# zjucsxxd/hdr2yuv

Hardware: AMD Instinct MI355X
Metric: Mpixels/s, 4K RGB->YUV420 PQ convert path (in-memory, HBM-resident) (higher is better)
Workload: dtype f32+f64

## Files before the change

hdr2yuv_amd/csrc/h2y_device.h:

```cpp
#ifndef H2Y_DEVICE_H
#define H2Y_DEVICE_H

#include <hip/hip_runtime.h>
#include <stdint.h>

#include "h2y_kernels.h"
#include "h2y_math.h"

using namespace h2y;

#define WAVE 64

__device__ __forceinline__ float wave_min(float v)
{
#pragma unroll
    for (int o = 32; o > 0; o >>= 1) v = fminf(v, __shfl_xor(v, o, WAVE));
    return v;
}
__device__ __forceinline__ float wave_max(float v)
{
#pragma unroll
    for (int o = 32; o > 0; o >>= 1) v = fmaxf(v, __shfl_xor(v, o, WAVE));
    return v;
}
// ... 219 lines not shown
{
    const uint32_t xb = f2bits(x);
    const bool cand = slow && (xb - 0x00800000u) < (lo_bits - 0x00800000u);
    if (__builtin_expect(__builtin_amdgcn_ballot_w64(cand) != 0 && ext != nullptr, 0)) {
        const uint32_t idx = cand ? (xb >> H2Y_PQ_LOW_BITS) - H2Y_PQX_SEG_BASE : 0u;
        const pq_ext_rec *X = reinterpret_cast<const pq_ext_rec *>(ext);
        const pq_recA a = X[idx].a;
        const pq_recB b = X[idx].b;
        const double d = pq_poly(xb, a, b);
        v = cand ? (float)d : v;
        slow = cand ? pq_ambiguous(d) : slow;
    }
    return v;
}

static __device__ __attribute__((noinline)) float tf_to_linear_careful(int cls, float v) { return tf_to_linear(cls, v); }
static __device__ __attribute__((noinline)) float tf_from_linear_careful(int cls, float v) { return tf_from_linear(cls, v); }

#define H2Y_PIPE_RUNTIME 0
#define H2Y_PIPE_PQ_IDENT 1
#define H2Y_PIPE_PQ_NORM 2
#define H2Y_PIPE_NONE 6
#define H2Y_PIPE_TFN 7

template <int PIPE> __device__ __forceinline__ float norm1(const pix_params &pp, int c, float v)
{
    const bool conv = PIPE == H2Y_PIPE_RUNTIME ? pp.convert_transfer != 0 : true;
    const bool ident = PIPE == H2Y_PIPE_RUNTIME ? pp.norm_identity : PIPE == H2Y_PIPE_PQ_IDENT;
    return (conv && !ident) ? (v - pp.offset[c]) / pp.range[c] : v;
}
// ... 172 lines not shown
```

hdr2yuv_amd/csrc/h2y_fir_fused.hip:

```cpp
#include <hip/hip_runtime.h>
#include <stdint.h>

#include <stdio.h>

#include "h2y_device.h"

#define FF_THREADS 1024
#ifndef FF_BUFFER_STORE
#define FF_BUFFER_STORE 1
#endif
#define FF_OWN_LANES H2Y_FF_OWN_LANES
#define FF_HALO ((64 - FF_OWN_LANES) / 2)

template <bool RAW> struct ff_rows;
template <> struct ff_rows<false> { float g0[4], b0[4], r0[4], g1[4], b1[4], r1[4]; };
template <> struct ff_rows<true> { uint32_t g0[2], b0[2], r0[2], g1[2], b1[2], r1[2]; };
template <int IN_KIND> __device__ __forceinline__ void ff_load(const void *p, uint32_t q, float (&d)[4]) { in_traits<IN_KIND>::load4q(p, q, d); }
template <int IN_KIND> __device__ __forceinline__ void ff_load(const void *p, uint32_t q, uint32_t (&d)[2])
{
    const u32x2 t = gload_nt<u32x2>(p, q);
    d[0] = t.x; d[1] = t.y;
}
__device__ __forceinline__ uint32_t ff_pk_min_h(uint32_t a, uint32_t b) { uint32_t r; asm("v_pk_min_f16 %0, %1, %2" : "=v"(r) : "v"(a), "v"(b)); return r; }
__device__ __forceinline__ uint32_t ff_pk_max_h(uint32_t a, uint32_t b) { uint32_t r; asm("v_pk_max_f16 %0, %1, %2" : "=v"(r) : "v"(a), "v"(b)); return r; }
// ... 155 lines not shown
        const uint32_t qx = (uint32_t)min(max(qxu, 0), (int32_t)WQ - 1);
        const bool own = lane >= (uint32_t)FF_HALO && lane < (uint32_t)FF_HALO + FF_OWN_LANES && qxu < (int32_t)WQ;
#if FF_BUFFER_STORE
        const uint32_t qx_store = own ? qx : 0x20000000u;
        const __amdgpu_buffer_rsrc_t out_rsrc = __builtin_amdgcn_make_buffer_rsrc(io.out, 0, (int)((npix + 2u * ncb) * 2u), 0x00020000);
#endif
        ff_edges e;
        e.any = __builtin_amdgcn_readfirstlane((uint32_t)(strip == 0u) | (uint32_t)(strip + 1u == nst));
        e.left0 = qxu == 0;
        e.left1 = qxu == 1;
        e.right0 = qxu == (int32_t)WQ - 1;

        mm6 mm;
        mm.reset();
        uint32_t flagged = 0;
        uint64_t low_m = 0;
        ff_hist hb[2], hr[2];
        hb[0].fill(0u); hb[1].fill(0u); hr[0].fill(0u); hr[1].fill(0u);

        constexpr bool RAW = TIER == FF_TIER_LUT16;
        constexpr int NREG = RAW ? 2 : 4;
        uint32_t hmn[3] = {0x7C007C00u, 0x7C007C00u, 0x7C007C00u}, hmx[3] = {0u, 0u, 0u};
        ff_rows<RAW> v;
        uint32_t q0 = 2u * (s_begin < H2 - 1u ? s_begin : H2 - 1u) * WQ + qx;
        ff_load<IN_KIND>(io.in[0], q0, v.g0); ff_load<IN_KIND>(io.in[1], q0, v.b0); ff_load<IN_KIND>(io.in[2], q0, v.r0);
        ff_load<IN_KIND>(io.in[0], q0 + WQ, v.g1); ff_load<IN_KIND>(io.in[1], q0 + WQ, v.b1); ff_load<IN_KIND>(io.in[2], q0 + WQ, v.r1);
#pragma unroll
        for (int j = 0; j < NREG; j++) asm volatile("" ::"v"(v.g0[j]), "v"(v.b0[j]), "v"(v.r0[j]), "v"(v.g1[j]), "v"(v.b1[j]), "v"(v.r1[j]));

        for (uint32_t s = s_begin; s <= s_end; s++) {
// ... 64 lines not shown
                    Y[col] = f2bits(gv[col]) >> 21; Cb[col] = f2bits(bv[col]) >> 21; Cr[col] = f2bits(rv[col]) >> 21;
                    continue;
#endif
                    const float Gn = norm1<PIPE>(pp, 0, gv[col]), Bn = norm1<PIPE>(pp, 1, bv[col]), Rn = norm1<PIPE>(pp, 2, rv[col]);
                    const pq_rec1 cg = pq_t1_fetch(Gn, s_t1), cb = pq_t1_fetch(Bn, s_t1), cr = pq_t1_fetch(Rn, s_t1);
                    __builtin_amdgcn_sched_barrier(0);
                    float mg, mb, mr;
                    const float g = pix_scale(pq_t1_eval_m(Gn, cg, &mg), pp.mulY, pp.addY);
                    const float b = pix_scale(pq_t1_eval_m(Bn, cb, &mb), pp.mulC, pp.addC);
                    const float rr = pix_scale(pq_t1_eval_m(Rn, cr, &mr), pp.mulC, pp.addC);
                    bool ra, rb;
                    pix_matrix_t1<MODE>(pp, sn, g, b, rr, pq_t1_unsure3(mg, mb, mr), Y[col], Cb[col], Cr[col], &ra, &rb);
                    const uint64_t fm = __builtin_amdgcn_ballot_w64(ra) | __builtin_amdgcn_ballot_w64(rb);
                    if (__builtin_expect(fm != 0, 0)) {
                        const bool ug = pq_t1_unsure(mg), ub = pq_t1_unsure(mb), ur = pq_t1_unsure(mr);
                        uint32_t Y2, Cb2, Cr2;
                        const bool fl = ((fm >> lane) & 1u) != 0;
                        float g2 = g, b2 = b, r2 = rr;
                        bool un = false;
                        if (__builtin_amdgcn_ballot_w64(fl & ug) != 0) {
                            bool sl;
                            const float t = pq_ext_inline(Gn, pq_fast(Gn, sA, sB, &sl), sl, pp.pq_ext);
                            g2 = (fl & ug) ? pix_scale(t, pp.mulY, pp.addY) : g2;
                            un |= fl & ug & sl;
                        }
                        if (__builtin_amdgcn_ballot_w64(fl & ub) != 0) {
                            bool sl;
                            const float t = pq_ext_inline(Bn, pq_fast(Bn, sA, sB, &sl), sl, pp.pq_ext);
                            b2 = (fl & ub) ? pix_scale(t, pp.mulC, pp.addC) : b2;
                            un |= fl & ub & sl;
                        }
                        if (__builtin_amdgcn_ballot_w64(fl & ur) != 0) {
                            bool sl;
                            const float t = pq_ext_inline(Rn, pq_fast(Rn, sA, sB, &sl), sl, pp.pq_ext);
                            r2 = (fl & ur) ? pix_scale(t, pp.mulC, pp.addC) : r2;
                            un |= fl & ur & sl;
                        }
                        bool um;
                        pix_matrix<MODE, false>(pp, g2, b2, r2, Y2, Cb2, Cr2, &um);
                        un |= um;
                        if (__builtin_expect(fl & un, 0)) {
                            const ycc k = pixel_careful<MODE>(&s_pp, Gn, Bn, Rn);
                            Y2 = k.y; Cb2 = k.cb; Cr2 = k.cr;
                        }
                        Y[col] = fl ? Y2 : Y[col];
                        Cb[col] = fl ? Cb2 - pp.half_m1 : Cb[col];
                        Cr[col] = fl ? Cr2 - pp.half_m1 : Cr[col];
                        flagged += (uint32_t)__popcll(fm);
                        if (PIPE == H2Y_PIPE_PQ_IDENT) low_m |= __builtin_amdgcn_ballot_w64(fl && min3f(Gn, Bn, Rn) <= -1.0f);
                    }
                    }
                }
                yp[row][0] = pix_yuv_clamp<true>(pp, Y[0], false) | (pix_yuv_clamp<true>(pp, Y[1], false) << 16);
                yp[row][1] = pix_yuv_clamp<true>(pp, Y[2], false) | (pix_yuv_clamp<true>(pp, Y[3], false) << 16);
#if defined(H2Y_EXP_NOCOMPUTE) && H2Y_EXP_NOCOMPUTE >= 2
                n_cb[row][0] = Cb[0]; n_cb[row][1] = Cb[2]; n_cr[row][0] = Cr[0]; n_cr[row][1] = Cr[2];
#else
                ff_hstage<TIER == FF_TIER_T1>(Cb, e, maxcv, hk0, n_cb[row][0], n_cb[row][1]);
                ff_hstage<TIER == FF_TIER_T1>(Cr, e, maxcv, hk0, n_cr[row][0], n_cr[row][1]);
#endif
                if (row == 0) {
                    ff_load<IN_KIND>(io.in[0], q0n, v.g0);
                    ff_load<IN_KIND>(io.in[1], q0n, v.b0);
                    ff_load<IN_KIND>(io.in[2], q0n, v.r0);
// ... 47 lines not shown
        if constexpr (RAW) {
#pragma unroll
            for (int c = 0; c < 3; c++) {
                mm.lo[c] = fminf(ff_half_to_float(hmn[c] & 0xFFFFu), ff_half_to_float(hmn[c] >> 16));
                mm.hi[c] = fmaxf(ff_half_to_float(hmx[c] & 0xFFFFu), ff_half_to_float(hmx[c] >> 16));
                mm.lo[c] = mm.lo[c] > 65504.0f ? 3.402823466e+38f : mm.lo[c];
                mm.hi[c] = mm.hi[c] <= 0.0f ? 1.175494351e-38f : mm.hi[c];
            }
        }
        asm volatile("" : "+s"(ap));
        const uint32_t f_end = __builtin_amdgcn_readfirstlane(u / ap->units_per_frame);
        const size_t slot = (size_t)u;
        wave_store_mm(mm, ap->partial + slot * 6);
        if (lane == 0) {
            ap->redo_count[slot] = flagged >> 3;
            if (PIPE == H2Y_PIPE_PQ_IDENT && ap->low_flag && low_m != 0) ap->low_flag[f_end] = 1u;
        }
    }
    if (a.block_clock && (threadIdx.x & (WAVE - 1)) == 0) atomicMax(&a.block_clock[2 * blockIdx.x + 1], (unsigned long long)wall_clock64());
#ifdef H2Y_BLOCK_TIMES
    if ((threadIdx.x & (WAVE - 1)) == 0) atomicMax(&g_ff_block_times[2 * blockIdx.x + 1], (unsigned long long)wall_clock64());
#endif
}

typedef void (*firf_fn)(firf_args);
template <int IN_KIND> static firf_fn pick_firf(int mode, int pipe)
{
    if (mode == H2Y_MODE_YCBCR)
        return pipe == H2Y_PIPE_PQ_IDENT ? k_fir_fused<IN_KIND, H2Y_MODE_YCBCR, H2Y_PIPE_PQ_IDENT, FF_TIER_T1>
                                         : k_fir_fused<IN_KIND, H2Y_MODE_YCBCR, H2Y_PIPE_PQ_NORM, FF_TIER_T1>;
// ... 16 lines not shown
```

hdr2yuv_amd/csrc/h2y_forward.hip:

```cpp
#include "h2y_shim.h"
#include "h2y_plan.h"

namespace {

const double kT1DenseShare = 0.007;
const double kFirSyncMaxFlagged = 0.004;
const int kT1SkipBatches = 32;
const int kT1SkipBatchesMax = 1024;

int tmp_depth_of(const h2y_desc *d) { return d->in_sample_type == H2Y_SAMPLE_U16 ? d->src_bit_depth : d->dst_bit_depth; }

}

void derive_params(const h2y_desc *d, pix_params *pp, bool stage_matrix_only)
{
    memset(pp, 0, sizeof *pp);
    const int tmp_depth = tmp_depth_of(d);
    const clip_limits tc = make_clip(tmp_depth, d->dst_full_range);
    const clip_limits oc = make_clip(d->dst_bit_depth, d->dst_full_range);
    pp->src_tf = tf_class(d->src_transfer);
    pp->dst_tf = tf_class(d->dst_transfer);
    if (d->src_transfer == d->dst_transfer) pp->convert_transfer = 0;
    else pp->convert_transfer = (pp->src_tf == H2Y_TF_LINEAR && pp->dst_tf == H2Y_TF_PQ) ? 1 : 2;
    pp->src_fn = pp->dst_fn = -1;
// ... 43 lines not shown
        }
    }
    pix_limits_finish(pp);
}

namespace {

void t1_begin_batch(h2y_ctx *ctx)
{
    ctx->cur_skip_t1 = ctx->t1_skip > 0;
    if (ctx->cur_skip_t1) ctx->t1_skip--;
}
void t1_end_batch(h2y_ctx *ctx, const h2y_desc *d, const frame_stats *fs, int n)
{
    if (!ctx->b->was_t1 || n < 1) return;
    uint64_t redone = 0;
    for (int f = 0; f < n; f++) redone += fs[f].redone;
    const uint64_t tiles = (uint64_t)n * make_geom(d->width, d->height, 1024).tiles;
    if (!strcmp(ctx->last_name, "k_fir_fused")) ctx->fir_flag_share = tiles ? (double)redone / (double)tiles : 0.0;
    {
        const size_t at = ctx->last_variant.find(" flagged=");
        if (at != std::string::npos) ctx->last_variant.erase(at);
        char note[48];
        snprintf(note, sizeof note, " flagged=%.5f", tiles ? (double)redone / (double)tiles : 0.0);
        ctx->last_variant += note;
    }
    if (ctx->opt_t1_steer && (double)redone > kT1DenseShare * (double)tiles) {
        ctx->t1_skip_len = ctx->t1_skip_len ? (ctx->t1_skip_len < kT1SkipBatchesMax ? 2 * ctx->t1_skip_len : kT1SkipBatchesMax) : kT1SkipBatches;
        ctx->t1_skip = ctx->t1_skip_len;
    } else ctx->t1_skip_len = 0;
}

fused_variant pick_variant(const h2y_ctx *ctx, const h2y_desc *d, const pix_params &pp, int out_kind, const assumed_stats *known, t1_sens *sn)
{
    memset(sn, 0, sizeof *sn);
    fused_variant v;
    v.in_kind = in_kind_of(d);
    v.out_kind = out_kind;
    v.mode = pp.mode;
    v.narrow = (d->width % 4) != 0;
    v.even_h = (d->height & 1) == 0;
    v.pipe = 0;
// ... 154 lines not shown
    fa.src_bit_depth = d->src_bit_depth;
    fa.redo_count = nullptr;
    fa.low_flag = nullptr;
    fa.check = 0;
    fa.assumed = nullptr;
    fa.publish = nullptr;
    fa.block_clock = nullptr;
    fa.grid = 0;
    fa.xcd_time = nullptr;
    return fa;
}
final_args launch_final(const h2y_ctx *ctx, const frames_run &r, int f0, int nblk, bool redo, bool low, bool clocks, int grid)
{
    final_args fa = stats_final(ctx, r.d, nblk, ctx->b->fs_out + r.fstats_offset + f0);
    fa.redo_count = redo ? ctx->b->d_redo : nullptr;
    fa.low_flag = low ? ctx->b->d_low : nullptr;
    fa.check = r.check ? 1 : 0;
    fa.assumed = r.d_assumed;
    fa.block_clock = clocks ? ctx->b->d_clock : nullptr;
    fa.grid = grid;
    static_assert(sizeof(frame_stats) >= 8 * sizeof(float), "the XCD run times ride in one frame_stats entry");
    fa.xcd_time = reinterpret_cast<float *>(ctx->b->fs_out + r.fstats_offset + r.n);
    return fa;
}

int stage_unit_rows(h2y_ctx *ctx, const std::vector<uint32_t> &rows)
{
    batch_state *b = ctx->b;
    const size_t units = rows.size();
    if (b->unit_rows_cap < units) {
// ... 16 lines not shown

int launch_fir_fused(h2y_ctx *ctx, const frames_run &r, const fir_plan &p)
{
    batch_state *b = ctx->b;
    const h2y_desc *d = r.d;
    const int n = r.n, grid = p.grid;
    const fused_variant &var = r.var;
    const bool ident = var.pipe == 4 || var.pipe == 3;
    const uint32_t upf = p.strips * p.segments;
    b->was_t1 = true;
    for (int i = 0; i < n; i++) b->h_frames[(size_t)ctx->slot_base + i] = r.frames[i];
    int rc = stage_frames(ctx, 0, n);
    if (rc) return rc;
    rc = ensure(ctx, b->d_partial, b->partial_cap, (size_t)n * upf * 6 * sizeof(float));
    if (rc) return rc;
    rc = ensure(ctx, b->d_redo, b->redo_cap, (size_t)n * upf * sizeof(uint32_t));
    if (rc) return rc;
    if (ident && (rc = ensure_low(ctx, n))) return rc;
    if (r.check) b->approx_min = ident;
    firf_args fa;
    fa.frames = b->d_frames + ctx->slot_base;
    fa.n_frames = n;
    fa.width = (uint32_t)d->width;
    fa.height = (uint32_t)d->height;
    fa.wq = p.wq;
    fa.n_strips = p.strips;
    fa.n_seg = p.segments;
    fa.seg_rows = p.seg_rows;
    fa.units_per_frame = upf;
    fa.total_units = (uint32_t)p.units;
    const int fsync = ctx->opt_fir_sync >= 0 ? ctx->opt_fir_sync : (ctx->fir_flag_share > kFirSyncMaxFlagged ? 0 : 1);
    fa.sync_mask = fsync > 0 ? (uint32_t)fsync - 1u : ~0u;
    fa.table = ctx->d_table;
    fa.table1 = ctx->d_table1;
    fa.lut16 = ctx->d_lut16;
    fa.sn = r.sn;
    fa.partial = b->d_partial;
    fa.redo_count = b->d_redo;
    fa.low_flag = ident ? b->d_low : nullptr;
    fa.assumed = r.d_assumed;
    fa.pp = r.pp;
    fa.unit_rows = nullptr;
    fa.block_clock = nullptr;
    fa.mix_xcds = p.mix_xcds;
    const bool clocks = p.full && r.time_it;
    const balance bal = balance_of(ctx);
    const bool weigh = fir_weigh(p, bal, ctx->ffb_have);
    double work[8] = {0, 0, 0, 0, 0, 0, 0, 0};
    if (weigh || clocks) {
        double sp[8];
        for (int x = 0; x < 8; x++) sp[x] = bal.speed(x, ctx->ffb_speed);
        std::vector<uint32_t> rows;
        fir_unit_rows(p, n, weigh, sp, rows, work);
// ... 67 lines not shown
    a.pp.tf_ext[0] = sf ? ctx->d_tfn_ext[sf] : nullptr;
    a.pp.tf_ext[1] = df ? ctx->d_tfn_ext[df] : nullptr;
    return 0;
}

int launch_fused(h2y_ctx *ctx, const frames_run &r, const geom &g, const launch_plan &l, int f0, bool first_launch, bool yuvp2)
{
    batch_state *b = ctx->b;
    const h2y_desc *d = r.d;
    const fused_variant &var = r.var;
    const int nf = l.frames, grid = l.grid, groups = l.groups;
    const int waves = h2y_fused_threads(var) / 64;
    int rc = ensure(ctx, b->d_partial, b->partial_cap, (size_t)nf * grid * waves * 6 * sizeof(float));
    if (rc) return rc;
    const bool t1 = var.pipe == 4 || var.pipe == 5;
    if (t1 && (rc = ensure(ctx, b->d_redo, b->redo_cap, (size_t)nf * grid * waves * sizeof(uint32_t)))) return rc;
    const bool approx = var.pipe == 4;
    if (approx && (rc = ensure_low(ctx, nf))) return rc;
    if (r.check) b->approx_min = approx;
    const uint32_t *d_slice_ranges = nullptr;
    slice_plan sl;
    for (int x = 0; x < 8; x++) sl.work[x] = 1;
    if (l.xcd_layout && ctx->opt_bal_mode != 1) {
        const balance bal = balance_of(ctx);
        double sp[8];
        for (int x = 0; x < 8; x++) sp[x] = bal.speed(x, ctx->bal_have ? ctx->bal_speed : nullptr);
        const block_speeds bs{ctx->opt_bal_mode == 0 && ctx->opt_bal_blocks, ctx->bal_bgrid, ctx->bal_bgroups, &ctx->bal_bspeed};
        make_slice_plan(sl, l, g.tiles, sp, bs, t1, ctx->opt_tail);
        if ((rc = publish_ranges(ctx, sl.r, first_launch, &d_slice_ranges))) return rc;
    }
    const bool clocks = l.xcd_layout && r.time_it;
// ... 2 lines not shown
    a.xcd_layout = l.xcd_layout ? 1u : 0u;
    a.block_clock = clocks ? b->d_clock : nullptr;
    a.slice_ranges = d_slice_ranges;
    a.range_stride = sl.range_stride;
    a.tail_ctr = nullptr;
    a.tail_slices = 0;
    if (sl.tail_on && d_slice_ranges) {
        if (!b->d_tail) {
            HIP_TRY(ctx, hipMalloc((void **)&b->d_tail, 16 * H2Y_TAIL_WORDS * sizeof(uint32_t)));
            HIP_TRY(ctx, hipMemsetAsync(b->d_tail, 0, 16 * H2Y_TAIL_WORDS * sizeof(uint32_t), ctx->stream));
        }
        a.tail_ctr = b->d_tail;
        a.tail_slices = sl.slices;
    }
    a.redo_count = t1 ? b->d_redo : nullptr;
    a.low_flag = approx ? b->d_low : nullptr;
    a.frames = b->d_frames + ctx->slot_base + f0;
    a.n_frames = nf;
    a.width = d->width;
    a.height = d->height;
    a.wq = g.wq;
    a.wq_magic = g.wq_magic;
    a.tiles_per_frame = g.tiles;
    a.chunks_per_frame = g.chunks;
    a.groups = (uint32_t)groups;
    a.table = ctx->d_table;
    a.table_src = a.table_dst = nullptr;
    a.lut16 = ctx->d_lut16;
    a.table1 = ctx->d_table1;
    a.sn = r.sn;
// ... 562 lines not shown
```

hdr2yuv_amd/csrc/h2y_kernels.h:

```cpp
#ifndef H2Y_KERNELS_H
#define H2Y_KERNELS_H

#include <hip/hip_runtime.h>
#include <stdint.h>

#include "h2y_math.h"
#include "h2y_walk.h"

#ifndef H2Y_FUSED_THREADS
#define H2Y_FUSED_THREADS 512
#endif
#ifndef H2Y_FUSED_MINWAVES
#define H2Y_FUSED_MINWAVES 4
#endif

#ifndef H2Y_LOOP_THREADS
#define H2Y_LOOP_THREADS 1024
#endif

#define H2Y_LUT16_N 16384

enum { H2Y_IN_F32 = 0, H2Y_IN_F16 = 1, H2Y_IN_U16 = 2 };
enum { H2Y_OUT_420BOX = 0, H2Y_OUT_444 = 1, H2Y_OUT_444TMP = 2 };

// ... 1 lines not shown
    const void *in[3];
    uint16_t *out;
    union {
        uint16_t *tmp_cb;
        uint16_t *yuv;
    };
    uint16_t *tmp_cr;
};

struct frame_stats {
    float mm[6];
    int32_t floor_[3];
    int32_t ceil_[3];
    int32_t mismatch;
    uint32_t redone;
};

struct assumed_stats {
    int32_t floor_[3];
    int32_t ceil_[3];
};

struct fused_args {
    const frame_io *frames;
    int n_frames;
    uint32_t width, height;
    uint32_t wq;
    uint32_t wq_magic;
    uint32_t tiles_per_frame;
    uint32_t chunks_per_frame;
    uint32_t groups;
    uint32_t xcd_layout;
    unsigned long long *block_clock;
    const uint32_t *slice_ranges;
    uint32_t *tail_ctr = nullptr;
    uint32_t tail_slices = 0;
    uint32_t range_stride = 0;
    const void *table;
    const void *table_src, *table_dst;
    const float *lut16;
    const void *table1;
    h2y::t1_sens sn;
    uint32_t tiles_magic;
    float *partial;
    uint32_t *redo_count;
    uint32_t *low_flag;
    const assumed_stats *assumed;
    h2y::pix_params pp;
};

struct fused_variant {
    int in_kind, out_kind, mode;
    int pipe;
    bool narrow;
    bool even_h;
    bool t1_ok = false;
    bool cols8 = false;
};

struct stats_args {
    const void *in[3];
    size_t npix;
    int vec_ok;
    float *partial;
};

struct final_args {
    const float *partial;
    const uint32_t *redo_count;
    uint32_t *low_flag;
    int nblk;
    frame_stats *out;
    int is_u16, src_bit_depth;
    int check;
    const assumed_stats *assumed;
    assumed_stats *publish;
    unsigned long long *block_clock;
    int grid;
    float *xcd_time;
    float *block_time = nullptr;
    uint32_t *tail_ctr = nullptr;
    int tail_n = 0;
};

// ... 32 lines not shown
    uint32_t width, height;
    uint32_t wq;
    uint32_t n_strips;
    uint32_t n_seg, seg_rows;
    const uint32_t *unit_rows;
    unsigned long long *block_clock;
    uint32_t mix_xcds;
    uint32_t units_per_frame;
    uint32_t total_units;
    uint32_t sync_mask;
    const void *table, *table1;
    const float *lut16;
    h2y::t1_sens sn;
    float *partial;
    uint32_t *redo_count;
    uint32_t *low_flag;
    const assumed_stats *assumed;
    h2y::pix_params pp;
};

enum { UP_REPLICATE = 0, UP_FIR = 1, UP_FIR_TL = 2 };
struct up_args {
    const uint16_t *src0, *src1;
    uint16_t *dst0, *dst1;
    int width, height;
    int algorithm;
    float fmin, fmax;
};

struct inv420_args {
// ... 356 lines not shown
```

hdr2yuv_amd/csrc/h2y_kernels.hip:

```cpp
#include <hip/hip_runtime.h>
#include <stdint.h>
#include <string.h>
#include <stdio.h>

#include "h2y_math.h"
#include "h2y_kernels.h"
#include "h2y_walk.h"
#include "h2y_device.h"

struct tile_pos {
    uint32_t tt;
    uint32_t q0, q1;
    bool row1;
};
__device__ __forceinline__ tile_pos tile_locate(uint32_t tt, uint32_t W, uint32_t H, uint32_t WQ, uint32_t magic)
{
    tile_pos t;
    uint32_t cg;
    (void)udiv_magic(tt, WQ, magic, cg);
    t.tt = tt;
    t.q0 = 2u * tt - cg;
    t.row1 = tt < WQ * (H >> 1);
    t.q1 = t.row1 ? t.q0 + WQ : t.q0;
    return t;
// ... 672 lines not shown
    for (; fw.f < fw.n_frames; fw.advance(), fo++) {
        const int f = fw.f;
        const bool dyn = tail_ctr != nullptr && !fw.has_next();
        const bool dyn_n = tail_ctr != nullptr && fw.has_next() && f + 2 * (int)fw.NG >= fw.n_frames;
        uint32_t dyn_t0 = 0;
        asm volatile("" : "+s"(ap));
        const frame_io *const frames = ap->frames;
        const frame_io io = uniform_io(frames + f);
        typedef const __attribute__((address_space(4))) frame_io *frame_cptr;
        const frame_cptr io_next_p = (frame_cptr)(uintptr_t)(frames + (fw.has_next() ? f + (int)fw.NG : f));
        mm6 mm;
        mm.reset();
        const uint32_t id_base = (uint32_t)f * a.tiles_per_frame;
        uint32_t flagged_f = 0;
        uint32_t flagged_px = 0;
        wave_deal deal, deal_n;
        if (ranged) {
            deal.set_range(r_first, r_count);
            deal_n.set_range(r_first, r_count);
        } else {
            deal.set(fw, fw.k0, H2Y_T1_THREADS / WAVE);
            deal_n.set(fw, fw.k0_n, H2Y_T1_THREADS / WAVE);
        }
        if (dyn) {
            if (!hold) {
                tick = wave_claim(&s_tq[H2Y_TAIL_QLEN + 2], s_scratch, true);
                hold = dyn_tile0(tick, dyn_t0);
            } else dyn_t0 = dyn_carry;
        } else if (!hold) {
            tick = wave_claim(&s_claim[fo], s_scratch, true);
// ... 119 lines not shown
                        if (row == 1) { Y[col] = o.yp0[col >> 1] >> (16 * (col & 1)) & 0xFFFFu; Cb[col] = sb[col >> 1] >> 1; Cr[col] = sr[col >> 1] >> 1; continue; }
#endif
                        const float Gn = norm1<PIPE>(pp, 0, gv[col]);
                        const float Bn = norm1<PIPE>(pp, 1, bv[col]);
                        const float Rn = norm1<PIPE>(pp, 2, rv[col]);
                        const pq_rec1 cg = pq_t1_fetch(Gn, s_t1), cb = pq_t1_fetch(Bn, s_t1), cr = pq_t1_fetch(Rn, s_t1);
                        __builtin_amdgcn_sched_barrier(0);
                        float mg, mb, mr;
                        const float g = pix_scale(pq_t1_eval_m(Gn, cg, &mg), pp.mulY, pp.addY);
                        const float b = pix_scale(pq_t1_eval_m(Bn, cb, &mb), pp.mulC, pp.addC);
                        const float r = pix_scale(pq_t1_eval_m(Rn, cr, &mr), pp.mulC, pp.addC);
                        bool ra, rb;
                        pix_matrix_t1<MODE>(pp, sn, g, b, r, pq_t1_unsure3(mg, mb, mr), Y[col], Cb[col], Cr[col], &ra, &rb);
                        const uint64_t fm = __builtin_amdgcn_ballot_w64(ra) | __builtin_amdgcn_ballot_w64(rb);
                        if (__builtin_expect(fm != 0, 0)) {
                            const bool fl = ((fm >> lane) & 1u) != 0;
                            const bool ug = pq_t1_unsure(mg), ub = pq_t1_unsure(mb), ur = pq_t1_unsure(mr);
                            float g2 = g, b2 = b, r2 = r;
                            bool un = false;
                            if (__builtin_amdgcn_ballot_w64(fl & ug) != 0) {
                                bool sl;
                                const float t = pq_ext_inline(Gn, pq_fast(Gn, s_t2, sB2, &sl), sl, pp.pq_ext);
                                g2 = (fl & ug) ? pix_scale(t, pp.mulY, pp.addY) : g2;
                                un |= fl & ug & sl;
                            }
                            if (__builtin_amdgcn_ballot_w64(fl & ub) != 0) {
                                bool sl;
                                const float t = pq_ext_inline(Bn, pq_fast(Bn, s_t2, sB2, &sl), sl, pp.pq_ext);
                                b2 = (fl & ub) ? pix_scale(t, pp.mulC, pp.addC) : b2;
                                un |= fl & ub & sl;
                            }
                            if (__builtin_amdgcn_ballot_w64(fl & ur) != 0) {
                                bool sl;
                                const float t = pq_ext_inline(Rn, pq_fast(Rn, s_t2, sB2, &sl), sl, pp.pq_ext);
                                r2 = (fl & ur) ? pix_scale(t, pp.mulC, pp.addC) : r2;
                                un |= fl & ur & sl;
                            }
                            uint32_t Y2, Cb2, Cr2;
                            bool um;
                            pix_matrix<MODE, false>(pp, g2, b2, r2, Y2, Cb2, Cr2, &um);
                            Y[col] = fl ? Y2 : Y[col];
                            Cb[col] = fl ? Cb2 - pp.half_m1 : Cb[col];
                            Cr[col] = fl ? Cr2 - pp.half_m1 : Cr[col];
                            redo_m |= __builtin_amdgcn_ballot_w64(fl & (un | um));
                            flagged_px += (uint32_t)__popcll(fm);
                        }
                        asm volatile("" : "+s"(redo_m));
                    }
                    row_pack<OUT_KIND, true, true>(pp, row, Y, Cb, Cr, o, sb, sr);
                }
                tile_store<OUT_KIND>(io, t, W, H, o);
                v = nx;
                t_cur = t2;
                {
                    const uint64_t m = redo_m;
                    const bool flagged = ((m >> lane) & 1u) != 0;
                    const uint32_t below = __builtin_amdgcn_mbcnt_hi((uint32_t)(m >> 32), __builtin_amdgcn_mbcnt_lo((uint32_t)m, 0u));
                    my_list[flagged ? n_redo + below : (uint32_t)(H2Y_REDO_CAP - 1)] = id_base + umin32(tt, a.tiles_per_frame - 1u);
                    n_redo = __builtin_amdgcn_readfirstlane(n_redo + (uint32_t)__popcll(m));
                    flagged_f = __builtin_amdgcn_readfirstlane(flagged_f + (uint32_t)__popcll(m));
// ... 1 lines not shown
                more = kind == 1;
                tick = tick2;
                if (dyn) dyn_t0 = dyn_t0_next;
            } while (more && n_redo < WAVE);
            if (n_redo >= WAVE) {
                n_redo -= WAVE;
#ifndef H2Y_SKIP_REDO
                redo_pass<IN_KIND, OUT_KIND, MODE, PIPE>(&s_rc, &s_pp, s_t2, my_list, n_redo, WAVE);
                have = false;
#endif
            }
        }
        asm volatile("" : "+s"(ap));
        wave_store_mm(mm, ap->partial + walk_slot(fw, H2Y_T1_THREADS / WAVE) * 6);
        if (ap->redo_count && lane == 0) ap->redo_count[walk_slot(fw, H2Y_T1_THREADS / WAVE)] = flagged_f + (flagged_px >> 3);
    }
#ifdef H2Y_BLOCK_TIMES
    if (blockIdx.x < 4 && lane == 0) g_block_times[2 * (800 + blockIdx.x * 16 + wave)] = wall_clock64();
#endif
    if (n_redo) redo_pass<IN_KIND, OUT_KIND, MODE, PIPE>(&s_rc, &s_pp, s_t2, my_list, 0u, n_redo);
    block_clock_end(a);
#ifdef H2Y_BLOCK_TIMES
    __syncthreads();
    if (threadIdx.x == 0) g_block_times[2 * blockIdx.x + 1] = wall_clock64();
#endif
    (void)lane;
}

typedef _Float16 h2 __attribute__((ext_vector_type(2)));
__device__ __forceinline__ uint32_t pk_min_h(uint32_t a, uint32_t b)
// ... 251 lines not shown
            IN::load4(a.in[c], i * 4, v);
            mm.add2(c, v[0], v[1]);
            mm.add2(c, v[2], v[3]);
        }
    }
    for (size_t i = n4 * 4 + (size_t)blockIdx.x * blockDim.x + threadIdx.x; i < n; i += stride)
#pragma unroll
        for (int c = 0; c < 3; c++) mm.add(c, IN::load1(a.in[c], i));
    block_store_mm<H2Y_FUSED_THREADS / WAVE>(mm, s_red, a.partial + (size_t)blockIdx.x * 6);
}

#define H2Y_FINAL_THREADS 1024
__global__ __launch_bounds__(H2Y_FINAL_THREADS) void k_stats_final(final_args a)
{
    __shared__ float s_red[(H2Y_FINAL_THREADS / WAVE) * 6];
    __shared__ uint32_t s_cnt;
    __shared__ int s_start[1024], s_finish[1024], s_min[8];
    const int f = blockIdx.x;
    const float *p = a.partial + (size_t)f * a.nblk * 6;
    frame_stats *out = a.out + f;
    mm6 mm;
    mm.reset();
    uint32_t cnt = 0;
    for (int i = threadIdx.x; i < a.nblk; i += blockDim.x) {
#pragma unroll
        for (int c = 0; c < 3; c++) {
            mm.lo[c] = fminf(mm.lo[c], p[i * 6 + 2 * c]);
            mm.hi[c] = fmaxf(mm.hi[c], p[i * 6 + 2 * c + 1]);
        }
        if (a.redo_count) cnt += a.redo_count[(size_t)f * a.nblk + i];
    }
    int as_floor[3] = {0, 0, 0}, as_ceil[3] = {0, 0, 0};
    uint32_t low = 0;
    if (threadIdx.x == 0) {
        if (a.check)
            for (int c = 0; c < 3; c++) { as_floor[c] = a.assumed->floor_[c]; as_ceil[c] = a.assumed->ceil_[c]; }
        if (a.low_flag) low = a.low_flag[f];
    }
    const bool clocks = a.block_clock && f == 0;
    const int nb = min(a.grid, 1024);
    if (clocks) {
        const unsigned long long ref = a.block_clock[0];
        for (int b = (int)threadIdx.x; b < a.grid; b += (int)blockDim.x) {
            if (b < nb) {
                s_start[b] = (int)(long long)(a.block_clock[2 * b] - ref);
                s_finish[b] = (int)(long long)(a.block_clock[2 * b + 1] - ref);
            }
            a.block_clock[2 * b + 1] = 0ull;
        }
    }
    if (a.tail_ctr && f == 0)
        for (int i = (int)threadIdx.x; i < a.tail_n; i += (int)blockDim.x) a.tail_ctr[i] = 0u;
    if (threadIdx.x == 0) s_cnt = 0;
    __syncthreads();
    if (a.redo_count) {
#pragma unroll
        for (int o = WAVE / 2; o > 0; o >>= 1) cnt += (uint32_t)__shfl_xor((int)cnt, o, WAVE);
        if ((threadIdx.x & (WAVE - 1)) == 0) atomicAdd(&s_cnt, cnt);
    }
    block_store_mm<H2Y_FINAL_THREADS / WAVE>(mm, s_red, out->mm);
    if (threadIdx.x == 0) {
        out->redone = a.redo_count ? s_cnt : 0u;
        int bad = 0;
        for (int c = 0; c < 3; c++) {
            float lo = s_red[2 * c], hi = s_red[2 * c + 1];
            int fl, ce;
            if (a.is_u16) {
                fl = (int)lo;
                ce = (int)hi;
                const int D = 1 << (a.src_bit_depth - 8), SMin = D * 16;
                const int YMax = 219 * D + SMin, CMax = 224 * D + SMin;
                if (ce < YMax && ce > (YMax * 3) / 4) ce = YMax;
                if (ce < CMax && ce > (CMax * 3) / 4) ce = CMax;
            } else {
                lo = fminf(fmaxf(lo, -2147483648.0f), 2147483520.0f);
                hi = fminf(fmaxf(hi, -2147483648.0f), 2147483520.0f);
                fl = (int)lo;
// ... 379 lines not shown
```

hdr2yuv_amd/csrc/h2y_math.h:

```cpp
#ifndef H2Y_MATH_H
#define H2Y_MATH_H

#if defined(H2Y_EXP_NOCOMPUTE) || defined(H2Y_HALF_COMPUTE) || defined(H2Y_SKIP_REDO) || defined(H2Y_EXP_NOSTATS) || defined(H2Y_EXP_NOCONFLICT) || \
    defined(H2Y_BLOCK_TIMES)
#ifndef H2Y_EXPERIMENT
#error "timing-experiment variant requested without -DH2Y_EXPERIMENT: this would build a product library with wrong bytes or debug output"
#endif
#endif

#include <stdint.h>
#include <vector>

#if defined(__HIPCC__)
#define H2Y_FN __host__ __device__ __forceinline__
#define H2Y_FN_NOINLINE __host__ __device__ inline __attribute__((noinline))
#else
#define H2Y_FN inline
#define H2Y_FN_NOINLINE inline __attribute__((noinline))
#endif

namespace h2y {

H2Y_FN uint32_t f2bits(float f) { return __builtin_bit_cast(uint32_t, f); }
H2Y_FN float bits2f(uint32_t u) { return __builtin_bit_cast(float, u); }
// ... 778 lines not shown
                dd num = dd_add(ev[j], dd{-ev[j - 1].hi, -ev[j - 1].lo});
                ev[j] = dd_div(num, dd{wn[j] - wn[j - lvl], 0.0});
            }
        const dd q2 = ev[2];
        const dd q1 = dd_add(ev[1], dd_mul_d(q2, -(wn[0] + wn[1])));
        const dd q0 = dd_add(dd_add(ev[0], dd_mul_d(ev[1], -wn[0])), dd_mul_d(q2, wn[0] * wn[1]));
        const double r = (double)(2 << H2Y_T1_SEG_BITS);
        const float c = (float)q0.hi;
        o.cb = bits2f(f2bits(c) + 1u);
        o.c0 = (float)((((q0.hi - (double)c) + q0.lo) * inv_u - 0.5) + (double)H2Y_T1_DELTA);
        o.c1 = (float)(q1.hi * r * inv_u);
        o.c2 = (float)(q2.hi * r * r * inv_u);
    }
    T[0] = T[H2Y_T1_NSEG + 1] = nan_rec;
}
enum : int { H2Y_MODE_IDENTITY = 0, H2Y_MODE_YDZDX = 1, H2Y_MODE_YCBCR = 2, H2Y_MODE_YPQRS = 3, H2Y_MODE_YUVP2 = 4 };

struct pix_params {
    int convert_transfer;
    int src_tf, dst_tf;
    int src_fn, dst_fn;
    int norm_identity;
    float offset[3], range[3];
    float mulY, addY, mulC, addC;
    int mode;
    double kr, kg, kb;
    double dcb, dcr;
    double inv_dcb, inv_dcr;
    float P, Q, RR, S;
    uint32_t half_m1;
// ... 163 lines not shown
    Cro = (uint32_t)sat_i32_f64(qr);
    const uint32_t fb = (uint32_t)(d2bits(fract_f64(qb)) >> 32), fr = (uint32_t)(d2bits(fract_f64(qr)) >> 32);
    const bool y_unsafe = !(__builtin_fabsf(fract_f32(ylike) - 0.5f) < sn.ty);
    const bool guard = vunc & (((fb - sn.cb_lo) >= sn.cb_span) | ((fr - sn.cr_lo) >= sn.cr_span));
    *ra = guard | (vunc & y_unsafe);
    *rb = false;
}
template <int MODE>
H2Y_FN bool pix_matrix_t1(const pix_params &pp, const t1_sens &sn, float G, float B, float R, bool vunc, uint32_t &Yo,
                          uint32_t &Cbo, uint32_t &Cro)
{
    bool ra, rb;
    pix_matrix_t1<MODE>(pp, sn, G, B, R, vunc, Yo, Cbo, Cro, &ra, &rb);
    return ra | rb;
}

H2Y_FN uint32_t hiword_of(double v) { return (uint32_t)(d2bits(v) >> 32); }
inline bool t1_chroma_in_range(const pix_params &pp)
{
    const double vhi = pq_exact_dd(dd{(double)H2Y_T1_DOMAIN_HI, 0.0}).hi * (1.0 + 1e-6), vlo = pq_exact_dd(dd{(double)H2Y_T1_DOMAIN_LO, 0.0}).hi * (1.0 - 1e-6);
    auto span = [&](double mul, double add, double *lo, double *hi) {
        const double a = add + mul * vlo, b = add + mul * vhi;
        *lo = (a < b ? a : b) - 1e-3 - 1e-6 * __builtin_fabs(a < b ? a : b);
        *hi = (a < b ? b : a) + 1e-3 + 1e-6 * __builtin_fabs(a < b ? b : a);
    };
    double glo, ghi, clo, chi;
    span(pp.mulY, pp.addY, &glo, &ghi);
    span(pp.mulC, pp.addC, &clo, &chi);
    double qlo[2], qhi[2];
    if (pp.mode == H2Y_MODE_YCBCR) {
// ... 180 lines not shown
```

hdr2yuv_amd/csrc/h2y_shim.h:

```cpp
#pragma once

#include <hip/hip_runtime.h>

#include <cmath>
#include <cstdarg>
#include <cstdio>
#include <cstdlib>
#include <algorithm>
#include <cstring>
#include <memory>
#include <new>
#include <string>
#include <vector>

#include "../../include/hdr2yuv_hip.h"
#include "h2y_kernels.h"
#include "h2y_math.h"

using namespace h2y;

#pragma GCC visibility push(hidden)

struct clip_limits {
    uint32_t minCV, maxCV, minVR, maxVR, minVRC, maxVRC, Half;
// ... 72 lines not shown
    int planes_check(h2y_ctx *ctx, const h2y_desc *d) const;
    uint64_t payload_bytes() const;
    uintptr_t align() const;
    hipError_t launch(const h2y_ctx *ctx, const payload_frame *frames, int n) const;
    const char *kernel() const;
    std::string variant() const;
};

struct batch_state {
    frame_io *d_frames = nullptr, *h_frames = nullptr;
    size_t frames_cap = 0;
    std::vector<frame_io> dev_frames;
    float *d_partial = nullptr;
    size_t partial_cap = 0;
    uint32_t *d_redo = nullptr;
    size_t redo_cap = 0;
    uint32_t *d_low = nullptr;
    size_t low_cap = 0;
    bool approx_min = false;
    unsigned long long *d_clock = nullptr;
    size_t clock_cap = 0;
    int bal_slot = 0;
    bool bal_pending = false;
    double bal_work[8] = {1, 1, 1, 1, 1, 1, 1, 1};
    uint32_t *h_ranges = nullptr, *hd_ranges = nullptr;
    uint32_t *d_tail = nullptr;
    float *h_btime = nullptr, *hd_btime = nullptr;
    int bal_grid = 0, bal_groups = 0;
    std::vector<double> bal_bwork;
    std::vector<uint32_t> range_slot[2];
// ... 323 lines not shown
```

Measured before the change: 375,900.

## Settle dark-pixel flagged lanes with a float PQ approximation before slow path

Adds a float-only PQ evaluation for very dark inputs (log2/exp2 polynomials plus a Newton reciprocal) that settles flagged pixels in the tier-1 and fused FIR kernels. When the result's error bound is safe, these pixels skip the slow double-precision extension path and are no longer counted as redone. The dark counts are tracked separately and reported through stats_final. The host steering heuristic changes to use a separate FIR dense threshold that ignores dark-settled pixels, so fewer batches fall back away from tier-1. It adds register pressure and extra ballots on the rare flagged path.

```diff
diff --git a/hdr2yuv_amd/csrc/h2y_device.h b/hdr2yuv_amd/csrc/h2y_device.h
--- a/hdr2yuv_amd/csrc/h2y_device.h
+++ b/hdr2yuv_amd/csrc/h2y_device.h
@@ -257,6 +257,32 @@
     return v;
 }
 
+template <int MODE>
+__device__ __forceinline__ uint64_t t1_dark_settle(const pix_params &pp, const t1_sens &sn, uint64_t fm, uint32_t lane, float Gn, float Bn, float Rn,
+                                                   bool ug, bool ub, bool ur, float g, float b, float r, uint32_t &Y, uint32_t &Cb, uint32_t &Cr,
+                                                   uint64_t *settled)
+{
+    const bool fl = ((fm >> lane) & 1u) != 0;
+    const bool dg = pq_is_dark(Gn), db = pq_is_dark(Bn), dr = pq_is_dark(Rn);
+    *settled = 0;
+    if (__builtin_amdgcn_ballot_w64(fl & (dg | db | dr)) == 0) return fm;
+    float gA = g, bA = b, rA = r;
+    if (__builtin_amdgcn_ballot_w64(fl & dg) != 0) gA = dg ? pix_scale(pq_dark(Gn), pp.mulY, pp.addY) : g;
+    if (__builtin_amdgcn_ballot_w64(fl & db) != 0) bA = db ? pix_scale(pq_dark(Bn), pp.mulC, pp.addC) : b;
+    if (__builtin_amdgcn_ballot_w64(fl & dr) != 0) rA = dr ? pix_scale(pq_dark(Rn), pp.mulC, pp.addC) : r;
+    uint32_t Y2, Cb2, Cr2;
+    bool ra, rb;
+    pix_matrix_t1<MODE>(pp, sn, gA, bA, rA, true, Y2, Cb2, Cr2, &ra, &rb);
+    const bool other = (ug & !dg) | (ub & !db) | (ur & !dr);
+    const bool fin = fl & (dg | db | dr) & !other & !(ra | rb) & t1_chroma_raw_ok(pp, Cb2) & t1_chroma_raw_ok(pp, Cr2);
+    Y = fin ? Y2 : Y;
+    Cb = fin ? Cb2 : Cb;
+    Cr = fin ? Cr2 : Cr;
+    const uint64_t fin_m = __builtin_amdgcn_ballot_w64(fin);
+    *settled = fin_m;
+    return fm & ~fin_m;
+}
+
 static __device__ __attribute__((noinline)) float tf_to_linear_careful(int cls, float v) { return tf_to_linear(cls, v); }
 static __device__ __attribute__((noinline)) float tf_from_linear_careful(int cls, float v) { return tf_from_linear(cls, v); }
 
diff --git a/hdr2yuv_amd/csrc/h2y_fir_fused.hip b/hdr2yuv_amd/csrc/h2y_fir_fused.hip
--- a/hdr2yuv_amd/csrc/h2y_fir_fused.hip
+++ b/hdr2yuv_amd/csrc/h2y_fir_fused.hip
@@ -193,6 +193,7 @@
         mm6 mm;
         mm.reset();
         uint32_t flagged = 0;
+        uint32_t dark_px = 0;
         uint64_t low_m = 0;
         ff_hist hb[2], hr[2];
         hb[0].fill(0u); hb[1].fill(0u); hr[0].fill(0u); hr[1].fill(0u);
@@ -287,8 +288,12 @@
                     const uint64_t fm = __builtin_amdgcn_ballot_w64(ra) | __builtin_amdgcn_ballot_w64(rb);
                     if (__builtin_expect(fm != 0, 0)) {
                         const bool ug = pq_t1_unsure(mg), ub = pq_t1_unsure(mb), ur = pq_t1_unsure(mr);
+                        uint64_t dark_m;
+                        const uint64_t fm2 = t1_dark_settle<MODE>(pp, sn, fm, lane, Gn, Bn, Rn, ug, ub, ur, g, b, rr, Y[col], Cb[col], Cr[col], &dark_m);
+                        dark_px += (uint32_t)__popcll(dark_m);
+                        if (fm2 != 0) {
                         uint32_t Y2, Cb2, Cr2;
-                        const bool fl = ((fm >> lane) & 1u) != 0;
+                        const bool fl = ((fm2 >> lane) & 1u) != 0;
                         float g2 = g, b2 = b, r2 = rr;
                         bool un = false;
                         if (__builtin_amdgcn_ballot_w64(fl & ug) != 0) {
@@ -319,8 +324,9 @@
                         Y[col] = fl ? Y2 : Y[col];
                         Cb[col] = fl ? Cb2 - pp.half_m1 : Cb[col];
                         Cr[col] = fl ? Cr2 - pp.half_m1 : Cr[col];
-                        flagged += (uint32_t)__popcll(fm);
+                        flagged += (uint32_t)__popcll(fm2);
                         if (PIPE == H2Y_PIPE_PQ_IDENT) low_m |= __builtin_amdgcn_ballot_w64(fl && min3f(Gn, Bn, Rn) <= -1.0f);
+                        }
                     }
                     }
                 }
@@ -398,6 +404,7 @@
         wave_store_mm(mm, ap->partial + slot * 6);
         if (lane == 0) {
             ap->redo_count[slot] = flagged >> 3;
+            if (ap->dark_count) ap->dark_count[slot] = ((flagged + dark_px) >> 3) - (flagged >> 3);
             if (PIPE == H2Y_PIPE_PQ_IDENT && ap->low_flag && low_m != 0) ap->low_flag[f_end] = 1u;
         }
     }
diff --git a/hdr2yuv_amd/csrc/h2y_forward.hip b/hdr2yuv_amd/csrc/h2y_forward.hip
--- a/hdr2yuv_amd/csrc/h2y_forward.hip
+++ b/hdr2yuv_amd/csrc/h2y_forward.hip
@@ -3,7 +3,9 @@
 
 namespace {
 
-const double kT1DenseShare = 0.007;
+const double kT1DenseShare = 0.010;
+const double kFirDenseShare = 0.003;
+const double kFirDarkKeep = 0.10;
 const double kFirSyncMaxFlagged = 0.004;
 const int kT1SkipBatches = 32;
 const int kT1SkipBatchesMax = 1024;
@@ -81,18 +83,22 @@
 void t1_end_batch(h2y_ctx *ctx, const h2y_desc *d, const frame_stats *fs, int n)
 {
     if (!ctx->b->was_t1 || n < 1) return;
-    uint64_t redone = 0;
-    for (int f = 0; f < n; f++) redone += fs[f].redone;
+    uint64_t redone = 0, dark = 0;
+    for (int f = 0; f < n; f++) { redone += fs[f].redone; dark += fs[f].dark; }
     const uint64_t tiles = (uint64_t)n * make_geom(d->width, d->height, 1024).tiles;
-    if (!strcmp(ctx->last_name, "k_fir_fused")) ctx->fir_flag_share = tiles ? (double)redone / (double)tiles : 0.0;
+    if (!strcmp(ctx->last_name, "k_fir_fused")) ctx->fir_flag_share = tiles ? (double)(redone + dark) / (double)tiles : 0.0;
     {
         const size_t at = ctx->last_variant.find(" flagged=");
         if (at != std::string::npos) ctx->last_variant.erase(at);
-        char note[48];
-        snprintf(note, sizeof note, " flagged=%.5f", tiles ? (double)redone / (double)tiles : 0.0);
+        char note[80];
+        int len = snprintf(note, sizeof note, " flagged=%.5f", tiles ? (double)(redone + dark) / (double)tiles : 0.0);
+        if (tiles && 2000 * dark >= tiles) snprintf(note + len, sizeof note - (size_t)len, " dark=%.3f", (double)dark / (double)tiles);
         ctx->last_variant += note;
     }
-    if (ctx->opt_t1_steer && (double)redone > kT1DenseShare * (double)tiles) {
+    const bool fir = !strcmp(ctx->last_name, "k_fir_fused");
+    const bool dense = fir ? (double)redone > kFirDenseShare * (double)tiles && (double)dark < kFirDarkKeep * (double)tiles
+                           : (double)redone > kT1DenseShare * (double)tiles;
+    if (ctx->opt_t1_steer && dense) {
         ctx->t1_skip_len = ctx->t1_skip_len ? (ctx->t1_skip_len < kT1SkipBatchesMax ? 2 * ctx->t1_skip_len : kT1SkipBatchesMax) : kT1SkipBatches;
         ctx->t1_skip = ctx->t1_skip_len;
     } else ctx->t1_skip_len = 0;
@@ -277,6 +283,7 @@
 {
     final_args fa = stats_final(ctx, r.d, nblk, ctx->b->fs_out + r.fstats_offset + f0);
     fa.redo_count = redo ? ctx->b->d_redo : nullptr;
+    fa.dark_count = redo ? ctx->b->d_dark : nullptr;
     fa.low_flag = low ? ctx->b->d_low : nullptr;
     fa.check = r.check ? 1 : 0;
     fa.assumed = r.d_assumed;
@@ -323,8 +330,9 @@
     if (rc) return rc;
     rc = ensure(ctx, b->d_partial, b->partial_cap, (size_t)n * upf * 6 * sizeof(float));
     if (rc) return rc;
-    rc = ensure(ctx, b->d_redo, b->redo_cap, (size_t)n * upf * sizeof(uint32_t));
-    if (rc) return rc;
+    rc = ensure(ctx, b->d_redo, b->redo_cap, 2 * (size_t)n * upf * sizeof(uint32_t));
+    if (rc) return rc;
+    b->d_dark = b->d_redo + (size_t)n * upf;
     if (ident && (rc = ensure_low(ctx, n))) return rc;
     if (r.check) b->approx_min = ident;
     firf_args fa;
@@ -346,6 +354,7 @@
     fa.sn = r.sn;
     fa.partial = b->d_partial;
     fa.redo_count = b->d_redo;
+    fa.dark_count = b->d_dark;
     fa.low_flag = ident ? b->d_low : nullptr;
     fa.assumed = r.d_assumed;
     fa.pp = r.pp;
@@ -443,7 +452,8 @@
     int rc = ensure(ctx, b->d_partial, b->partial_cap, (size_t)nf * grid * waves * 6 * sizeof(float));
     if (rc) return rc;
     const bool t1 = var.pipe == 4 || var.pipe == 5;
-    if (t1 && (rc = ensure(ctx, b->d_redo, b->redo_cap, (size_t)nf * grid * waves * sizeof(uint32_t)))) return rc;
+    if (t1 && (rc = ensure(ctx, b->d_redo, b->redo_cap, 2 * (size_t)nf * grid * waves * sizeof(uint32_t)))) return rc;
+    if (t1) b->d_dark = b->d_redo + (size_t)nf * grid * waves;
     const bool approx = var.pipe == 4;
     if (approx && (rc = ensure_low(ctx, nf))) return rc;
     if (r.check) b->approx_min = approx;
@@ -476,6 +486,7 @@
         a.tail_slices = sl.slices;
     }
     a.redo_count = t1 ? b->d_redo : nullptr;
+    a.dark_count = t1 ? b->d_dark : nullptr;
     a.low_flag = approx ? b->d_low : nullptr;
     a.frames = b->d_frames + ctx->slot_base + f0;
     a.n_frames = nf;
diff --git a/hdr2yuv_amd/csrc/h2y_kernels.h b/hdr2yuv_amd/csrc/h2y_kernels.h
--- a/hdr2yuv_amd/csrc/h2y_kernels.h
+++ b/hdr2yuv_amd/csrc/h2y_kernels.h
@@ -39,6 +39,7 @@
     int32_t ceil_[3];
     int32_t mismatch;
     uint32_t redone;
+    uint32_t dark;
 };
 
 struct assumed_stats {
@@ -69,6 +70,7 @@
     uint32_t tiles_magic;
     float *partial;
     uint32_t *redo_count;
+    uint32_t *dark_count = nullptr;
     uint32_t *low_flag;
     const assumed_stats *assumed;
     h2y::pix_params pp;
@@ -93,6 +95,7 @@
 struct final_args {
     const float *partial;
     const uint32_t *redo_count;
+    const uint32_t *dark_count = nullptr;
     uint32_t *low_flag;
     int nblk;
     frame_stats *out;
@@ -155,6 +158,7 @@
     h2y::t1_sens sn;
     float *partial;
     uint32_t *redo_count;
+    uint32_t *dark_count = nullptr;
     uint32_t *low_flag;
     const assumed_stats *assumed;
     h2y::pix_params pp;
diff --git a/hdr2yuv_amd/csrc/h2y_kernels.hip b/hdr2yuv_amd/csrc/h2y_kernels.hip
--- a/hdr2yuv_amd/csrc/h2y_kernels.hip
+++ b/hdr2yuv_amd/csrc/h2y_kernels.hip
@@ -710,6 +710,7 @@
         const uint32_t id_base = (uint32_t)f * a.tiles_per_frame;
         uint32_t flagged_f = 0;
         uint32_t flagged_px = 0;
+        uint32_t dark_px = 0;
         wave_deal deal, deal_n;
         if (ranged) {
             deal.set_range(r_first, r_count);
@@ -859,8 +860,12 @@
                         pix_matrix_t1<MODE>(pp, sn, g, b, r, pq_t1_unsure3(mg, mb, mr), Y[col], Cb[col], Cr[col], &ra, &rb);
                         const uint64_t fm = __builtin_amdgcn_ballot_w64(ra) | __builtin_amdgcn_ballot_w64(rb);
                         if (__builtin_expect(fm != 0, 0)) {
-                            const bool fl = ((fm >> lane) & 1u) != 0;
                             const bool ug = pq_t1_unsure(mg), ub = pq_t1_unsure(mb), ur = pq_t1_unsure(mr);
+                            uint64_t dark_m;
+                            const uint64_t fm2 = t1_dark_settle<MODE>(pp, sn, fm, lane, Gn, Bn, Rn, ug, ub, ur, g, b, r, Y[col], Cb[col], Cr[col], &dark_m);
+                            dark_px += (uint32_t)__popcll(dark_m);
+                            if (fm2 != 0) {
+                            const bool fl = ((fm2 >> lane) & 1u) != 0;
                             float g2 = g, b2 = b, r2 = r;
                             bool un = false;
                             if (__builtin_amdgcn_ballot_w64(fl & ug) != 0) {
@@ -888,7 +893,8 @@
                             Cb[col] = fl ? Cb2 - pp.half_m1 : Cb[col];
                             Cr[col] = fl ? Cr2 - pp.half_m1 : Cr[col];
                             redo_m |= __builtin_amdgcn_ballot_w64(fl & (un | um));
-                            flagged_px += (uint32_t)__popcll(fm);
+                            flagged_px += (uint32_t)__popcll(fm2);
+                            }
                         }
                         asm volatile("" : "+s"(redo_m));
                     }
@@ -920,6 +926,7 @@
         asm volatile("" : "+s"(ap));
         wave_store_mm(mm, ap->partial + walk_slot(fw, H2Y_T1_THREADS / WAVE) * 6);
         if (ap->redo_count && lane == 0) ap->redo_count[walk_slot(fw, H2Y_T1_THREADS / WAVE)] = flagged_f + (flagged_px >> 3);
+        if (ap->dark_count && lane == 0) ap->dark_count[walk_slot(fw, H2Y_T1_THREADS / WAVE)] = ((flagged_px + dark_px) >> 3) - (flagged_px >> 3);
     }
 #ifdef H2Y_BLOCK_TIMES
     if (blockIdx.x < 4 && lane == 0) g_block_times[2 * (800 + blockIdx.x * 16 + wave)] = wall_clock64();
@@ -1201,14 +1208,14 @@
 __global__ __launch_bounds__(H2Y_FINAL_THREADS) void k_stats_final(final_args a)
 {
     __shared__ float s_red[(H2Y_FINAL_THREADS / WAVE) * 6];
-    __shared__ uint32_t s_cnt;
+    __shared__ uint32_t s_cnt, s_dark;
     __shared__ int s_start[1024], s_finish[1024], s_min[8];
     const int f = blockIdx.x;
     const float *p = a.partial + (size_t)f * a.nblk * 6;
     frame_stats *out = a.out + f;
     mm6 mm;
     mm.reset();
-    uint32_t cnt = 0;
+    uint32_t cnt = 0, dark = 0;
     for (int i = threadIdx.x; i < a.nblk; i += blockDim.x) {
 #pragma unroll
         for (int c = 0; c < 3; c++) {
@@ -1216,6 +1223,7 @@
             mm.hi[c] = fmaxf(mm.hi[c], p[i * 6 + 2 * c + 1]);
         }
         if (a.redo_count) cnt += a.redo_count[(size_t)f * a.nblk + i];
+        if (a.dark_count) dark += a.dark_count[(size_t)f * a.nblk + i];
     }
     int as_floor[3] = {0, 0, 0}, as_ceil[3] = {0, 0, 0};
     uint32_t low = 0;
@@ -1238,16 +1246,22 @@
     }
     if (a.tail_ctr && f == 0)
         for (int i = (int)threadIdx.x; i < a.tail_n; i += (int)blockDim.x) a.tail_ctr[i] = 0u;
-    if (threadIdx.x == 0) s_cnt = 0;
+    if (threadIdx.x == 0) s_cnt = s_dark = 0;
     __syncthreads();
     if (a.redo_count) {
 #pragma unroll
         for (int o = WAVE / 2; o > 0; o >>= 1) cnt += (uint32_t)__shfl_xor((int)cnt, o, WAVE);
         if ((threadIdx.x & (WAVE - 1)) == 0) atomicAdd(&s_cnt, cnt);
+    }
+    if (a.dark_count) {
+#pragma unroll
+        for (int o = WAVE / 2; o > 0; o >>= 1) dark += (uint32_t)__shfl_xor((int)dark, o, WAVE);
+        if ((threadIdx.x & (WAVE - 1)) == 0) atomicAdd(&s_dark, dark);
     }
     block_store_mm<H2Y_FINAL_THREADS / WAVE>(mm, s_red, out->mm);
     if (threadIdx.x == 0) {
         out->redone = a.redo_count ? s_cnt : 0u;
+        out->dark = a.dark_count ? s_dark : 0u;
         int bad = 0;
         for (int c = 0; c < 3; c++) {
             float lo = s_red[2 * c], hi = s_red[2 * c + 1];
diff --git a/hdr2yuv_amd/csrc/h2y_math.h b/hdr2yuv_amd/csrc/h2y_math.h
--- a/hdr2yuv_amd/csrc/h2y_math.h
+++ b/hdr2yuv_amd/csrc/h2y_math.h
@@ -816,6 +816,58 @@
     }
     T[0] = T[H2Y_T1_NSEG + 1] = nan_rec;
 }
+#define H2Y_DARK_HI_BITS 0x33800000u
+#define H2Y_DARK_LO_BITS 0x0D800000u
+#define H2Y_DARK_ERR 9.7e-9f
+static_assert(H2Y_DARK_ERR <= 0x1p-24f, "the first tier's windows cover a move of 2^-23 per sample; the dark estimate may use half");
+H2Y_FN float dark_exp2(float t)
+{
+    const float r = t + 0x1.8p23f;
+    const int32_t ti = (int32_t)(f2bits(r) - 0x4B400000u);
+    const float f = t - (r - 0x1.8p23f);
+    float e = 0x1.446c7ep-13f;
+    e = __builtin_fmaf(e, f, 0x1.5f48c8p-10f);
+    e = __builtin_fmaf(e, f, 0x1.3b29d8p-7f);
+    e = __builtin_fmaf(e, f, 0x1.c6aeccp-5f);
+    e = __builtin_fmaf(e, f, 0x1.ebfbe0p-3f);
+    e = __builtin_fmaf(e, f, 0x1.62e430p-1f);
+    e = __builtin_fmaf(e, f, 1.0f);
+    return bits2f(f2bits(e) + ((uint32_t)ti << 23));
+}
+H2Y_FN float pq_dark(float x)
+{
+    const uint32_t b = f2bits(x);
+    const uint32_t k = b - 0x3F3504F3u;
+    const int32_t ex = (int32_t)k >> 23;
+    const float g = bits2f((k & 0x007FFFFFu) + 0x3F3504F3u) - 1.0f;
+    float l = -0x1.2b6cc2p-3f;
+    l = __builtin_fmaf(l, g, 0x1.dfa96ap-3f);
+    l = __builtin_fmaf(l, g, -0x1.fd964ap-3f);
+    l = __builtin_fmaf(l, g, 0x1.25f726p-2f);
+    l = __builtin_fmaf(l, g, -0x1.70e346p-2f);
+    l = __builtin_fmaf(l, g, 0x1.ec775ap-2f);
+    l = __builtin_fmaf(l, g, -0x1.715526p-1f);
+    l = __builtin_fmaf(l, g, 0x1.715474p+0f);
+    const float m1 = 0.1593017578125f;
+    const float t = __builtin_fmaf(l * g, m1, (float)ex * m1);
+    const float p = dark_exp2(t);
+    const float den = __builtin_fmaf(18.6875f, p, 1.0f);
+    const float num = __builtin_fmaf(-0.1640625f, p, 0.1640625f);
+    float r = bits2f(0x7EF311C7u - f2bits(den));
+    r = __builtin_fmaf(r, __builtin_fmaf(-den, r, 1.0f), r);
+    r = __builtin_fmaf(r, __builtin_fmaf(-den, r, 1.0f), r);
+    r = __builtin_fmaf(r, __builtin_fmaf(-den, r, 1.0f), r);
+    float d = num * r;
+    d = __builtin_fmaf(__builtin_fmaf(-den, d, num), r, d);
+    float q = -0x1.e63be8p-2f;
+    q = __builtin_fmaf(q, d, -0x1.436d7ep-2f);
+    q = __builtin_fmaf(q, d, -0x1.f189fcp-2f);
+    q = __builtin_fmaf(q, d, -0x1.713208p-1f);
+    q = __builtin_fmaf(q, d, -0x1.7154d0p+0f);
+    const float v = dark_exp2(78.84375f * (q * d));
+    return b < H2Y_DARK_LO_BITS ? bits2f(H2Y_PQ_AT_ZERO_BITS) : v;
+}
+H2Y_FN bool pq_is_dark(float x) { return f2bits(x) < H2Y_DARK_HI_BITS; }
 enum : int { H2Y_MODE_IDENTITY = 0, H2Y_MODE_YDZDX = 1, H2Y_MODE_YCBCR = 2, H2Y_MODE_YPQRS = 3, H2Y_MODE_YUVP2 = 4 };
 
 struct pix_params {
@@ -1009,6 +1061,8 @@
     pix_matrix_t1<MODE>(pp, sn, G, B, R, vunc, Yo, Cbo, Cro, &ra, &rb);
     return ra | rb;
 }
+
+H2Y_FN bool t1_chroma_raw_ok(const pix_params &pp, uint32_t raw) { return raw + pp.half_m1 <= pp.maxCV; }
 
 H2Y_FN uint32_t hiword_of(double v) { return (uint32_t)(d2bits(v) >> 32); }
 inline bool t1_chroma_in_range(const pix_params &pp)
diff --git a/hdr2yuv_amd/csrc/h2y_shim.h b/hdr2yuv_amd/csrc/h2y_shim.h
--- a/hdr2yuv_amd/csrc/h2y_shim.h
+++ b/hdr2yuv_amd/csrc/h2y_shim.h
@@ -110,6 +110,7 @@
     float *d_partial = nullptr;
     size_t partial_cap = 0;
     uint32_t *d_redo = nullptr;
+    uint32_t *d_dark = nullptr;
     size_t redo_cap = 0;
     uint32_t *d_low = nullptr;
     size_t low_cap = 0;
```

Result: slower. 371,300 (-1.2%).
